# gregspangenberg/shoulder

Measured on AMD Instinct MI355X. Metric: humerus meshes/s end-to-end (all 4 landmarks), higher is better.
Workload: dtype f64 geometry + bf16 UNet

## Files before the change

shoulder_amd/csrc/k_slices.h:

```cpp
#pragma once
#include "sh_demand.h"
#include "sh_scalar.h"
#include "sh_cutmath.h"

namespace sh {

struct __attribute__((aligned(16))) Seg {
  uint32_t s_lo, s_hi, e_lo, e_hi;
};
static_assert(sizeof(Seg) == 16, "Seg must be 16 bytes");
__device__ inline void seg_start_point(const double* __restrict__ vb , uint32_t lo, uint32_t hi, double z, double* x, double* y) {
  const double* pl = vb + 3 * (size_t)lo;
  const double* ph = vb + 3 * (size_t)hi;
  const double dl = pl[2] - z, dh = ph[2] - z;
  const double t = dl / (dl - dh);
  *x = pl[0] + t * (ph[0] - pl[0]);
  *y = pl[1] + t * (ph[1] - pl[1]);
}

__device__ inline unsigned long long enc_f64(double v) {
  unsigned long long b = (unsigned long long)__double_as_longlong(v);
  return (b & 0x8000000000000000ull) ? ~b : (b | 0x8000000000000000ull);
}
__device__ inline double dec_f64(unsigned long long e) {
  unsigned long long b = (e & 0x8000000000000000ull) ? (e & 0x7FFFFFFFFFFFFFFFull) : ~e;
  return __longlong_as_double((long long)b);
}

__global__ void k_transform_verts(const float* __restrict__ verts, const long long* __restrict__ voff,
                                  const double* __restrict__ T, double* __restrict__ vobb,
                                  unsigned long long* __restrict__ zb_enc ) {
  int b = blockIdx.y;
  long long v0 = voff[b], nv = voff[b + 1] - v0;
  const double* Tb = T + 16 * b;
  double zmin = 1e300, zmax = -1e300;
  for (long long i = blockIdx.x * (long long)blockDim.x + threadIdx.x; i < nv; i += (long long)gridDim.x * blockDim.x) {
    const float* p = verts + 3 * (v0 + i);
    double o[3];
    xform_pt(Tb, (double)p[0], (double)p[1], (double)p[2], o);
    double* q = vobb + 3 * (v0 + i);
    q[0] = o[0]; q[1] = o[1]; q[2] = o[2];
    zmin = fmin(zmin, o[2]); zmax = fmax(zmax, o[2]);
  }
  for (int off = 32; off > 0; off >>= 1) {
    zmin = fmin(zmin, __shfl_down(zmin, off));
    zmax = fmax(zmax, __shfl_down(zmax, off));
  }
  if ((threadIdx.x & 63) == 0) {
    atomicMin(&zb_enc[2 * b], enc_f64(zmin));
    atomicMin(&zb_enc[2 * b + 1], ~enc_f64(zmax));
  }
}

__global__ void k_decode_bounds(const unsigned long long* zb_enc, double* zb, int B) {
  int i = blockIdx.x * blockDim.x + threadIdx.x;
  if (i < 2 * B) zb[i] = dec_f64((i & 1) ? ~zb_enc[i] : zb_enc[i]);
}

__device__ inline double np_pairwise_sum(const double* a, int n) {
  if (n < 8) {
    double r = 0.0;
    for (int i = 0; i < n; ++i) r += a[i];
    return r;
  } else if (n <= 128) {
    double r[8];
    for (int k = 0; k < 8; ++k) r[k] = a[k];
    int i;
    for (i = 8; i < n - (n % 8); i += 8)
      for (int k = 0; k < 8; ++k) r[k] += a[i + k];
    double res = ((r[0] + r[1]) + (r[2] + r[3])) + ((r[4] + r[5]) + (r[6] + r[7]));
    for (; i < n; ++i) res += a[i];
    return res;
  } else {
    int n2 = n / 2;
    n2 -= n2 % 8;
    return np_pairwise_sum(a, n2) + np_pairwise_sum(a + n2, n - n2);
  }
}

struct PlaneAux {
  const unsigned long long* zb_enc; double* zb_out;
  int* seg_count; int* nlarge;
  int* ovf_nlist; unsigned long long* ovf_ctr;
};
struct ManyLoops { int* list; int* n; unsigned long long* missed; };
struct SliceSetDev {
  int N, kind, select;
  const double* zb;
  double* zs; double* zeff;
  int* seg_count; Seg* segs;
  double* centroids; double* areas; int* nloops; int* ring_n; double* ring ; double* areas_total ;
  int* nlarge; ManyLoops many; unsigned long long* ovf_missed;
  PlaneAux aux;
};
struct OpenCfg { int mode; double max_gap; int* stats; };

struct SliceSets { SliceSetDev s[2]; int n; const double* vobb; const long long* voff; OpenCfg open; };

__global__ void k_make_planes(SliceSets sets, const double* __restrict__ neck_z, int B) {
  const SliceSetDev& S = sets.s[blockIdx.y];
  const int kind = S.kind, N = S.N;
  const double* zb = S.zb;
  double* zs = S.zs; double* zeff = S.zeff;
  const PlaneAux A = S.aux;
  int b = blockIdx.x;
  if (b >= B) return;
  for (int k = threadIdx.x; k < N; k += blockDim.x) A.seg_count[(size_t)b * N + k] = 0;
  if (b == 0 && threadIdx.x == 0) {
    *A.nlarge = 0;
    if (A.ovf_nlist) { A.ovf_nlist[0] = 0; A.ovf_nlist[1] = 0 ; if (A.ovf_ctr) { A.ovf_ctr[SH_CTR_SEG_USED] = 0ull; A.ovf_ctr[SH_CTR_WORK_USED] = 0ull; } }
  }
  if (kind == 3) {
    if (threadIdx.x == 0) { zs[b] = neck_z[b]; zeff[b] = neck_z[b]; }
    return;
  }
  double zmin, zmax;
  if (A.zb_enc) {
    zmin = dec_f64(A.zb_enc[2 * b]); zmax = dec_f64(~A.zb_enc[2 * b + 1]);
    if (threadIdx.x == 0) { A.zb_out[2 * b] = zmin; A.zb_out[2 * b + 1] = zmax; }
  } else { zmin = zb[2 * b]; zmax = zb[2 * b + 1]; }
  double a, e;
  if (kind == 4) {
    for (int k = threadIdx.x; k < N; k += blockDim.x) { double z = linspace_at(zmin * 0.99, zmax * 0.99, N, k); zs[(size_t)b * N + k] = z; zeff[(size_t)b * N + k] = z; }
    return;
  }
  if (kind == 0) { a = 0.99 * zmax; e = 0.99 * zmin; }
  else if (kind == 1) { a = 0.99 * zmax; e = neck_z[b]; }
  else { a = 0.99 * zmin; e = 0.0; }
  double* z = zs + (size_t)b * N;
  for (int k = threadIdx.x; k < N; k += blockDim.x) z[k] = linspace_at(a, e, N, k);
  __syncthreads();
  __shared__ double z_orig;
  if (threadIdx.x == 0) z_orig = np_pairwise_sum(z, N) / (double)N;
  __syncthreads();
  for (int k = threadIdx.x; k < N; k += blockDim.x) zeff[(size_t)b * N + k] = z_orig + (z[k] - z_orig);
}

#define SH_EMIT_MAXN 640
__global__ void __launch_bounds__(256)
k_slice_emit(const double* __restrict__ vobb, const int* __restrict__ faces,
             const long long* __restrict__ voff, const long long* __restrict__ foff, SliceSets sets) {
  __shared__ int hist[SH_EMIT_MAXN];
  int b = blockIdx.y;
  long long f0 = foff[b], nf = foff[b + 1] - f0;
  const double* vb = vobb + 3 * voff[b];
  const int nsets = sets.n, Ntot = sets.s[0].N + (nsets > 1 ? sets.s[1].N : 0);
  for (long long f_base = blockIdx.x * (long long)blockDim.x; f_base < nf; f_base += (long long)gridDim.x * blockDim.x) {
    for (int k = threadIdx.x; k < Ntot; k += blockDim.x) hist[k] = 0;
    const long long fi = f_base + threadIdx.x;
    const bool live = fi < nf;
    const int* f = faces + 3 * (f0 + (live ? fi : 0));
    int id[3] = {f[0], f[1], f[2]};
    double Z[3];
    for (int k = 0; k < 3; ++k) Z[k] = vb[3 * (size_t)id[k] + 2];
    double fzmin = fmin(Z[0], fmin(Z[1], Z[2])), fzmax = fmax(Z[0], fmax(Z[1], Z[2]));
    int lo_[2] = {1, 1}, hi_[2] = {0, 0};
    for (int si = 0; si < nsets; ++si) {
      const int N = sets.s[si].N;
      const double* zp = sets.s[si].zeff + (size_t)b * N;
      const double z_first = zp[0], z_last = zp[N - 1];
      const double inv_step = (double)(N - 1) / (z_last - z_first);
      double ka = (fzmin - z_first) * inv_step, kb = (fzmax - z_first) * inv_step;
      double klo = fmin(ka, kb), khi = fmax(ka, kb);
      int lo = 1, hi = 0;
      if (live && !(khi < -1.0 || klo > (double)N)) {
        lo = (int)floor(fmax(klo, 0.0)) - 1; hi = (int)ceil(fmin(khi, (double)(N - 1))) + 1;
        lo = lo < 0 ? 0 : lo;
        hi = hi > N - 1 ? N - 1 : hi;
      }
      if (live && N == 1) { lo = 0; hi = 0; }
      lo_[si] = lo; hi_[si] = hi;
    }
    __syncthreads();
    for (int si = 0; si < nsets; ++si) {
      const int N = sets.s[si].N, hoff = si ? sets.s[0].N : 0;
      const double* zp = sets.s[si].zeff + (size_t)b * N;
      for (int k = lo_[si]; k <= hi_[si]; ++k) {
        const double z = zp[k];
        const int s0 = Z[0] - z < -SH_SECTION_TOL ? -1 : 1, s1 = Z[1] - z < -SH_SECTION_TOL ? -1 : 1, s2 = Z[2] - z < -SH_SECTION_TOL ? -1 : 1;
        if (!(s0 == s1 && s1 == s2)) atomicAdd(&hist[hoff + k], 1);
      }
    }
    __syncthreads();
    for (int k = threadIdx.x; k < Ntot; k += blockDim.x) {
      const int n = hist[k];
      if (n > 0) {
        const int si = k >= sets.s[0].N ? 1 : 0, kk = si ? k - sets.s[0].N : k;
        hist[k] = atomicAdd(&sets.s[si].seg_count[(size_t)b * sets.s[si].N + kk], n);
      }
    }
    __syncthreads();
    for (int si = 0; si < nsets; ++si) {
      const int N = sets.s[si].N, hoff = si ? sets.s[0].N : 0;
      const double* zp = sets.s[si].zeff + (size_t)b * N;
      Seg* segs = sets.s[si].segs;
      for (int k = lo_[si]; k <= hi_[si]; ++k) {
        const double z = zp[k];
        double d[3];
        int s[3];
        for (int j = 0; j < 3; ++j) { d[j] = Z[j] - z; s[j] = d[j] < -SH_SECTION_TOL ? -1 : 1; }
        if (s[0] == s[1] && s[1] == s[2]) continue;
        const int slot = atomicAdd(&hist[hoff + k], 1);
        int up = 0, dn = 0;
        for (int j = 0; j < 3; ++j) {
          int jn = (j + 1) % 3;
          if (s[j] == -1 && s[jn] == 1) up = j;
          if (s[j] == 1 && s[jn] == -1) dn = j;
        }
        Seg sg;
        {
          int a = dn, c = (dn + 1) % 3;
          int l = id[a] < id[c] ? a : c, h = id[a] < id[c] ? c : a;
          sg.s_lo = (uint32_t)id[l]; sg.s_hi = (uint32_t)id[h];
        }
        {
          int a = up, c = (up + 1) % 3;
          int l = id[a] < id[c] ? a : c, h = id[a] < id[c] ? c : a;
          sg.e_lo = (uint32_t)id[l]; sg.e_hi = (uint32_t)id[h];
        }
        if (slot < SH_MAXSEG) segs[((size_t)b * N + k) * SH_MAXSEG + slot] = sg;
      }
    }
    __syncthreads();
  }
}

#define SH_LINK_THREADS 256
#define SH_SMALLSEG 384

template <int T>
__device__ inline int bridge_open_chains(const int n, const int cap, const int maxe, unsigned long long* __restrict__ skey,
                                         const unsigned long long* __restrict__ ekey, int* __restrict__ nxt, int* __restrict__ pred,
                                         int* __restrict__ ctl, int* tl, int* hd, int* bt, int* bh, int* mt, int* mh,
                                         double* tx, double* ty, double* hx, double* hy,
                                         const double* __restrict__ vb, const double z, const double max_gap) {
  const int tid = threadIdx.x;
  for (int i = tid; i < n; i += T) pred[i] = 0;
  if (tid < 4) ctl[tid] = 0;
  __syncthreads();
  for (int i = tid; i < n; i += T) if (nxt[i] != i) atomicAdd(&pred[nxt[i]], 1);
  __syncthreads();
  for (int i = tid; i < n; i += T) {
    if (nxt[i] == i) { const int q = atomicAdd(&ctl[0], 1); if (q < maxe) tl[q] = i; }
    if (pred[i] == 0) { const int q = atomicAdd(&ctl[1], 1); if (q < maxe) hd[q] = i; }
  }
  __syncthreads();
  const int nt = ctl[0], nh = ctl[1];
  if (nt > maxe || nh > maxe) return -1;
  for (int q = tid; q < nt; q += T) { const unsigned long long k = ekey[tl[q]]; seg_start_point(vb, (uint32_t)(k >> 32), (uint32_t)k, z, &tx[q], &ty[q]); mt[q] = -1; }
  for (int q = tid; q < nh; q += T) { const unsigned long long k = skey[hd[q]]; seg_start_point(vb, (uint32_t)(k >> 32), (uint32_t)k, z, &hx[q], &hy[q]); mh[q] = -1; }
  for (;;) {
    __syncthreads();
    if (tid == 0) ctl[2] = 0;
    for (int q = tid; q < nt; q += T) {
      int best = -1; double bd = 0.0; unsigned long long bk = 0;
      if (mt[q] < 0)
        for (int h = 0; h < nh; ++h) {
          if (mh[h] >= 0) continue;
          const double dx = tx[q] - hx[h], dy = ty[q] - hy[h];
          const double d = sqrt(dx * dx + dy * dy);
          if (!(d <= max_gap)) continue;
          const unsigned long long k = skey[hd[h]];
          if (best < 0 || d < bd || (d == bd && k < bk)) { best = h; bd = d; bk = k; }
        }
      bt[q] = best;
    }
    for (int q = tid; q < nh; q += T) {
      int best = -1; double bd = 0.0; unsigned long long bk = 0;
      if (mh[q] < 0)
        for (int t = 0; t < nt; ++t) {
          if (mt[t] >= 0) continue;
          const double dx = tx[t] - hx[q], dy = ty[t] - hy[q];
          const double d = sqrt(dx * dx + dy * dy);
          if (!(d <= max_gap)) continue;
          const unsigned long long k = ekey[tl[t]];
          if (best < 0 || d < bd || (d == bd && k < bk)) { best = t; bd = d; bk = k; }
        }
      bh[q] = best;
    }
    __syncthreads();
    for (int q = tid; q < nt; q += T) {
      const int h = bt[q];
      if (h >= 0 && bh[h] == q) { mt[q] = h; mh[h] = q; ctl[2] = 1; }
    }
    __syncthreads();
    if (ctl[2] == 0) break;
  }
  for (int q = tid; q < nt; q += T)
    if (mt[q] >= 0) {
      const int v = n + atomicAdd(&ctl[3], 1);
      if (v < cap) { skey[v] = ekey[tl[q]]; nxt[v] = hd[mt[q]]; nxt[tl[q]] = v; }
    }
  __syncthreads();
  const int nb = ctl[3];
  return n + nb > cap ? -1 : n + nb;
}


template <int CAP, bool OPEN>
__device__ inline void slice_link_plane(const int pl, int N, const int* __restrict__ seg_count, const Seg* __restrict__ segs,
             const double* __restrict__ vobb, const long long* __restrict__ voff, const double* __restrict__ zeff,
             double* __restrict__ centroids, double* __restrict__ areas, int* __restrict__ nloops,
             int* __restrict__ ring_n, double* __restrict__ ring , int select, int* __restrict__ err,
             double* __restrict__ areas_total , ManyLoops many, const OpenCfg oc,
             int* __restrict__ nlarge = nullptr) {
  constexpr int HASH = CAP <= 384 ? 512 : 2048;
  static_assert(HASH * 4 <= CAP * 8 && HASH > CAP, "the hash table lives in bufB");
  __shared__ unsigned long long skey[CAP];
  __shared__ unsigned long long bufA[CAP];
  __shared__ unsigned long long bufB[CAP];
  __shared__ int nxt[CAP], jmpA[CAP], jmpB[CAP], offA[CAP], offB[CAP];
  int* const table = (int*)bufB;
  __shared__ unsigned long long l_key[SH_MAXLOOPS];
  __shared__ int l_start[SH_MAXLOOPS], l_len[SH_MAXLOOPS], l_off[SH_MAXLOOPS];
  __shared__ double l_area[SH_MAXLOOPS], l_sel[SH_MAXLOOPS];
  __shared__ int n_loops, bad;
  __shared__ double bbv[4];

  const int b = pl / N;
  const int tid = threadIdx.x;
  int cnt = seg_count[pl];
  if (CAP == SH_SMALLSEG ? cnt > SH_SMALLSEG : cnt <= SH_SMALLSEG) {
    if (CAP == SH_SMALLSEG && nlarge && tid == 0) atomicAdd(nlarge, 1);
    return;
  }
  if (cnt > SH_MAXSEG) return;
  const int n = cnt;
  if (tid == 0) { n_loops = 0; bad = 0; }
  for (int i = tid; i < HASH; i += SH_LINK_THREADS) table[i] = -1;
  const Seg* sp = segs + (size_t)pl * SH_MAXSEG;
  const double* vb = vobb + 3 * voff[b];
  const double zpl = zeff[pl];
  for (int i = tid; i < n; i += SH_LINK_THREADS) {
    Seg s = sp[i];
    skey[i] = ((unsigned long long)s.s_lo << 32) | s.s_hi;
    bufA[i] = ((unsigned long long)s.e_lo << 32) | s.e_hi;
  }
  __syncthreads();
  if (n < 3 && !(OPEN && n > 0)) {
    if (tid == 0) {
      centroids[2 * (size_t)pl] = 0; centroids[2 * (size_t)pl + 1] = 0; areas[pl] = 0; nloops[pl] = 0; ring_n[pl] = 0;
      if (areas_total) areas_total[pl] = 0;
      else atomicCAS(&err[b], 0, SH_ERR_GEOMETRY_DEV);
    }
    return;
  }
  for (int i = tid; i < n; i += SH_LINK_THREADS) {
    uint32_t h = hash_key64(skey[i]) & (HASH - 1);
    while (atomicCAS(&table[h], -1, i) != -1) h = (h + 1) & (HASH - 1);
  }
  __syncthreads();
  for (int i = tid; i < n; i += SH_LINK_THREADS) {
    unsigned long long k = bufA[i];
    uint32_t h = hash_key64(k) & (HASH - 1);
    int t, found = -1;
    while ((t = table[h]) != -1) {
      if (skey[t] == k) { found = t; break; }
      h = (h + 1) & (HASH - 1);
    }
    if (found < 0) { found = i; bad = 1; }
    nxt[i] = found;
  }
  __syncthreads();
  const bool bridging = OPEN && (bad || n < 3);
  int n2 = n;
  if (bridging) {
    constexpr int E = SH_MAXLOOPS;
    double* pts = (double*)bufB;
    n2 = bridge_open_chains<SH_LINK_THREADS>(n, CAP, E, skey, bufA, nxt, offB, jmpB, jmpA, jmpA + E, jmpA + 2 * E, jmpA + 3 * E, jmpA + 4 * E,
                                             jmpA + 5 * E, pts, pts + E, pts + 2 * E, pts + 3 * E, vb, zpl, oc.max_gap);
    if (n2 < 0) {
      if (tid == 0) {
        if (many.list) many.list[atomicAdd(many.n, 1)] = pl;
        else if (many.missed) atomicExch(many.missed, 1ull);
        else atomicExch(&err[b], SH_ERR_CAPACITY_DEV);
      }
      return;
    }
    if (tid == 0) bad = 0;
  }
  unsigned long long* labA = bufA;
  unsigned long long* labB = bufB;
  int* ja = jmpA; int* jb = jmpB;
  int* ra = offA; int* rb = offB;
  for (int i = tid; i < n2; i += SH_LINK_THREADS) { labA[i] = skey[i]; ja[i] = nxt[i]; ra[i] = 0; }
  __syncthreads();
  for (int span = 1; span < n2; span <<= 1) {
    for (int i = tid; i < n2; i += SH_LINK_THREADS) {
      const int j = ja[i];
      const unsigned long long a = labA[i], c = labA[j];
      const bool own = a <= c;
      labB[i] = own ? a : c;
      rb[i] = own ? ra[i] : span + ra[j];
      jb[i] = ja[j];
    }
    __syncthreads();
    unsigned long long* tl = labA; labA = labB; labB = tl;
    int* tj = ja; ja = jb; jb = tj;
    int* tr = ra; ra = rb; rb = tr;
  }
  for (int i = tid; i < n2; i += SH_LINK_THREADS)
    if (ra[i] == 0 && (!bridging || (nxt[ja[i]] != ja[i] && ra[nxt[i]] >= 2))) {
      int l = atomicAdd(&n_loops, 1);
      if (l < SH_MAXLOOPS) l_start[l] = i;
    }
  __syncthreads();
  if (n_loops > SH_MAXLOOPS) {
    if (tid == 0) {
      if (many.list) many.list[atomicAdd(many.n, 1)] = pl;
      else if (many.missed) atomicExch(many.missed, 1ull);
      else atomicExch(&err[b], SH_ERR_CAPACITY_DEV);
    }
    return;
  }
  const int nl = n_loops;
  if (tid == 0) {
    for (int a = 1; a < nl; ++a) {
      int v = l_start[a]; int c = a - 1;
      while (c >= 0 && skey[l_start[c]] > skey[v]) { l_start[c + 1] = l_start[c]; --c; }
      l_start[c + 1] = v;
    }
    int off = 0;
    for (int l = 0; l < nl; ++l) {
      int s = l_start[l];
      int L = ra[nxt[s]] + 1;
      l_len[l] = L; l_off[l] = off; off += L;
      l_key[l] = skey[s];
    }
    if (off != n && !bridging) bad = 1;
  }
  __syncthreads();
  if (bridging) {
    if (oc.stats)
      for (int i = tid; i < n; i += SH_LINK_THREADS)
        if (nxt[i] == i || nxt[i] >= n) {
          bool kept = false;
          for (int q = 0; q < nl; ++q) kept |= l_key[q] == labA[i];
          atomicAdd(&oc.stats[2 * b + (kept ? 0 : 1)], 1);
        }
    if (nl == 0) {
      if (tid == 0) {
        centroids[2 * (size_t)pl] = 0; centroids[2 * (size_t)pl + 1] = 0; areas[pl] = 0; nloops[pl] = 0; ring_n[pl] = 0;
        if (areas_total) areas_total[pl] = 0;
        else atomicCAS(&err[b], 0, SH_ERR_GEOMETRY_DEV);
      }
      return;
    }
    __syncthreads();
  }
  double* rx = (double*)bufA;
  double* ry = (double*)bufB;
  int my_pos[(CAP + SH_LINK_THREADS - 1) / SH_LINK_THREADS];
  {
    int c = 0;
    for (int i = tid; i < n2; i += SH_LINK_THREADS, ++c) {
      const unsigned long long key = labA[i];
      int l = -1;
      for (int q = 0; q < nl; ++q) if (l_key[q] == key) { l = q; break; }
      const int L = l >= 0 ? l_len[l] : 1;
      const int r = ra[i];
      const int pos = r == 0 ? 0 : L - r;
      my_pos[c] = l < 0 ? -1 : l_off[l] + pos;
    }
  }
  __syncthreads();
  {
    int c = 0;
    for (int i = tid; i < n2; i += SH_LINK_THREADS, ++c)
      if (my_pos[c] >= 0 && my_pos[c] < n2) {
        if (!OPEN || i < n) { const Seg sg = sp[i]; seg_start_point(vb, sg.s_lo, sg.s_hi, zpl, &rx[my_pos[c]], &ry[my_pos[c]]); }
        else { const unsigned long long kv = skey[i]; seg_start_point(vb, (uint32_t)(kv >> 32), (uint32_t)kv, zpl, &rx[my_pos[c]], &ry[my_pos[c]]); }
      }
  }
  __syncthreads();
  const int lane = tid & 63, wave = tid >> 6;
  const int nv = bridging ? l_off[nl - 1] + l_len[nl - 1] : n;
  if (wave == SH_LINK_THREADS / 64 - 1) {
    double x0 = 1e300, x1 = -1e300, y0 = 1e300, y1 = -1e300;
    for (int i = lane; i < nv; i += 64) {
      const double qx = rx[i], qy = ry[i];
      x0 = fmin(x0, qx); x1 = fmax(x1, qx); y0 = fmin(y0, qy); y1 = fmax(y1, qy);
    }
    for (int off = 32; off > 0; off >>= 1) {
      x0 = fmin(x0, __shfl_down(x0, off)); x1 = fmax(x1, __shfl_down(x1, off));
      y0 = fmin(y0, __shfl_down(y0, off)); y1 = fmax(y1, __shfl_down(y1, off));
    }
    if (lane == 0) { bbv[0] = x0; bbv[1] = x1; bbv[2] = y0; bbv[3] = y1; }
  } else {
    for (int l = wave; l < nl; l += SH_LINK_THREADS / 64 - 1) {
      const int o = l_off[l], L = l_len[l];
      double a2 = 0.0, mx = 0.0, my = 0.0;
      for (int q = lane; q < L; q += 64) {
        const int qn = q + 1 == L ? 0 : q + 1;
        a2 += rx[o + q] * ry[o + qn] - rx[o + qn] * ry[o + q];
        mx += rx[o + q]; my += ry[o + q];
      }
      for (int off = 32; off > 0; off >>= 1) { a2 += __shfl_down(a2, off); mx += __shfl_down(mx, off); my += __shfl_down(my, off); }
      if (lane == 0) {
        l_area[l] = 0.5 * a2;
        mx = (mx + rx[o]) / (double)(L + 1); my = (my + ry[o]) / (double)(L + 1);
        l_sel[l] = fabs(mx) + fabs(my);
      }
    }
  }
  __syncthreads();
  int best = 0;
  for (int l = 1; l < nl; ++l) {
    if (select == 0) { if (fabs(l_area[l]) > fabs(l_area[best])) best = l; }
    else { if (l_sel[l] < l_sel[best]) best = l; }
  }
  if (tid == 0) {
    double x0 = bbv[0], x1 = bbv[1], y0 = bbv[2], y1 = bbv[3];
    centroids[2 * (size_t)pl] = 0.5 * (x0 + x1);
    centroids[2 * (size_t)pl + 1] = 0.5 * (y0 + y1);
    int amax = 0;
    for (int l = 1; l < nl; ++l) if (fabs(l_area[l]) > fabs(l_area[amax])) amax = l;
    areas[pl] = fabs(l_area[amax]);
    if (areas_total) {
      double tot = 0.0;
      for (int l = 0; l < nl; ++l) tot += l_area[l];
      areas_total[pl] = fabs(tot);
    }
    nloops[pl] = nl;
    ring_n[pl] = l_len[best];
    if (bad) atomicCAS(&err[b], 0, SH_ERR_GEOMETRY_DEV);
  }
  if (ring) {
    int l = best, o = l_off[l], L = l_len[l];
    bool rev = l_area[l] < 0;
    double* out = ring + (size_t)pl * (SH_MAXSEG + 1) * 2;
    for (int q = tid; q <= L; q += SH_LINK_THREADS) {
      int qq = q == L ? 0 : q;
      int src = rev ? (qq == 0 ? 0 : L - qq) : qq;
      out[2 * q] = rx[o + src];
      out[2 * q + 1] = ry[o + src];
    }
  }
}

template <bool OPEN>
__global__ void __launch_bounds__(SH_LINK_THREADS)
k_slice_link(SliceSets sets, int B, int* __restrict__ err) {
  const int ntot = sets.s[0].N + (sets.n > 1 ? sets.s[1].N : 0);
  int id = (int)blockIdx.x;
  if (B % 8 == 0) { const int x = id & 7, j = id >> 3; id = (x + 8 * (j / ntot)) * ntot + j % ntot; }
  const int b = id / ntot, kk = id - b * ntot;
  const int si = kk >= sets.s[0].N ? 1 : 0;
  const SliceSetDev& S = sets.s[si];
  slice_link_plane<SH_SMALLSEG, OPEN>(b * S.N + (kk - (si ? sets.s[0].N : 0)), S.N, S.seg_count, S.segs, sets.vobb, sets.voff, S.zeff, S.centroids, S.areas, S.nloops, S.ring_n,
                                S.ring, S.select, err, S.areas_total, S.many, sets.open, S.nlarge);
}
template <bool OPEN>
__global__ void __launch_bounds__(SH_LINK_THREADS)
k_slice_link_large(SliceSets sets, int B, int* __restrict__ err) {
  for (int si = 0; si < sets.n; ++si) {
    const SliceSetDev& S = sets.s[si];
    if (*S.nlarge == 0) continue;
    const int nplanes = B * S.N;
    for (int pl = blockIdx.x; pl < nplanes; pl += gridDim.x) {
      const int cnt = S.seg_count[pl];
      if (cnt > SH_MAXSEG && S.ovf_missed && threadIdx.x == 0) atomicExch(S.ovf_missed, 1ull);
      if (cnt <= SH_SMALLSEG || cnt > SH_MAXSEG) continue;
      slice_link_plane<SH_MAXSEG, OPEN>(pl, S.N, S.seg_count, S.segs, sets.vobb, sets.voff, S.zeff, S.centroids, S.areas, S.nloops, S.ring_n, S.ring, S.select, err, S.areas_total, S.many, sets.open);
      __syncthreads();
    }
  }
}

#define SH_RS_THREADS 128
struct RsWant { int keep_all, st_lo, cs_lo, cs_hi; };
template <int CAP>
__device__ inline void resample_polar_plane(const int pl, int N, int M, const int* __restrict__ ring_n, const double* __restrict__ ring,
                 const double* __restrict__ centroids, double* __restrict__ ixy,
                 double* __restrict__ itr_start, double* __restrict__ itr_cs, const long long* __restrict__ ovf_roff, const RsWant W) {
  static_assert(SH_MPROX % SH_RS_THREADS == 0, "whole samples per lane");
  constexpr int NS = SH_MPROX / SH_RS_THREADS;
  __shared__ double rx[CAP + 1], ry[CAP + 1], d[CAP + 1];
  __shared__ int amin_idx;
  __shared__ double wmin[SH_RS_THREADS / 64];
  __shared__ int widx[SH_RS_THREADS / 64];
  const int tid = threadIdx.x;
  const int L = ring_n[pl];
  if (CAP == SH_SMALLSEG ? L > SH_SMALLSEG : L <= SH_SMALLSEG) return;
  if (ovf_roff[pl] >= 0) return;
  const int kpl = pl % N;
  const bool want_st = W.keep_all || kpl >= W.st_lo, want_cs = W.keep_all || (kpl >= W.cs_lo && kpl < W.cs_hi);
  if (!want_st && !want_cs) return;
  const double* rp = ring + (size_t)pl * (SH_MAXSEG + 1) * 2;
  for (int q = tid; q <= L; q += SH_RS_THREADS) { rx[q] = rp[2 * q]; ry[q] = rp[2 * q + 1]; }
  __syncthreads();
  for (int q = 1 + tid; q <= L; q += SH_RS_THREADS) {
    double dx = rx[q] - rx[q - 1], dy = ry[q] - ry[q - 1];
    d[q] = sqrt(dx * dx + dy * dy);
  }
  __syncthreads();
  if (tid == 0) {
    double acc = 0.0;
    d[0] = 0.0;
    int q = 1;
    for (; q + 8 <= L + 1; q += 8) {
      double v[8];
#pragma unroll
      for (int u = 0; u < 8; ++u) v[u] = d[q + u];
#pragma unroll
      for (int u = 0; u < 8; ++u) { acc += v[u]; v[u] = acc; }
#pragma unroll
      for (int u = 0; u < 8; ++u) d[q + u] = v[u];
    }
    for (; q <= L; ++q) { acc += d[q]; d[q] = acc; }
  }
  __syncthreads();
  const double dmax = d[L];
  double sx[NS], sy[NS];
#pragma unroll
  for (int u = 0; u < NS; ++u) {
    const int j = tid + u * SH_RS_THREADS;
    const double t = linspace_at(0.0, dmax, M, j);
    const int n = L + 1;
    if (t < d[0]) { sx[u] = rx[0]; sy[u] = ry[0]; }
    else if (!(t < d[n - 1])) { sx[u] = rx[n - 1]; sy[u] = ry[n - 1]; }
    else {
      int lo = 0, hi = n - 1;
      while (hi - lo > 1) { const int mid = (lo + hi) >> 1; if (t >= d[mid]) lo = mid; else hi = mid; }
      const double x0 = d[lo], fx = rx[lo], fy = ry[lo];
      if (x0 == t) { sx[u] = fx; sy[u] = fy; }
      else {
        const double den = d[lo + 1] - x0;
        sx[u] = (rx[lo + 1] - fx) / den * (t - x0) + fx;
        sy[u] = (ry[lo + 1] - fy) / den * (t - x0) + fy;
      }
    }
  }
  if (W.keep_all) {
    double* oxy = ixy + (size_t)pl * 2 * M;
#pragma unroll
    for (int u = 0; u < NS; ++u) { const int j = tid + u * SH_RS_THREADS; oxy[j] = sx[u]; oxy[M + j] = sy[u]; }
  }
  const double cx = centroids[2 * (size_t)pl], cy = centroids[2 * (size_t)pl + 1];
  for (int pass = 0; pass < 2; ++pass) {
    if (pass == 0 ? !want_st : !want_cs) continue;
    const double ox = pass ? cx : 0.0, oy = pass ? cy : 0.0;
    double best = 1e300;
    int bi = 0x7fffffff;
    double th[NS], rr[NS];
#pragma unroll
    for (int u = 0; u < NS; ++u) {
      const int j = tid + u * SH_RS_THREADS;
      const double x = sx[u] - ox, y = sy[u] - oy;
      th[u] = atan2(y, x);
      rr[u] = sqrt(x * x + y * y);
      if (th[u] < best || (th[u] == best && j < bi)) { best = th[u]; bi = j; }
    }
    for (int off = 32; off > 0; off >>= 1) {
      double ob = __shfl_down(best, off);
      int oi = __shfl_down(bi, off);
      if (ob < best || (ob == best && oi < bi)) { best = ob; bi = oi; }
    }
    if ((tid & 63) == 0) { wmin[tid >> 6] = best; widx[tid >> 6] = bi; }
    __syncthreads();
    if (tid == 0) {
      double bv = wmin[0]; int bx = widx[0];
      for (int w = 1; w < SH_RS_THREADS / 64; ++w)
        if (wmin[w] < bv || (wmin[w] == bv && widx[w] < bx)) { bv = wmin[w]; bx = widx[w]; }
      amin_idx = bx;
    }
    __syncthreads();
    const int k0 = amin_idx;
    double* o = (pass ? itr_cs : itr_start) + (size_t)pl * 2 * M;
#pragma unroll
    for (int u = 0; u < NS; ++u) {
      int dst = tid + u * SH_RS_THREADS - k0; if (dst < 0) dst += M;
      o[dst] = th[u];
      o[M + dst] = rr[u];
    }
    __syncthreads();
  }
}

__global__ void __launch_bounds__(SH_RS_THREADS)
k_resample_polar(int N, int M, const int* __restrict__ ring_n, const double* __restrict__ ring, const double* __restrict__ centroids,
                 double* __restrict__ ixy, double* __restrict__ itr_start, double* __restrict__ itr_cs, const long long* __restrict__ ovf_roff, const RsWant W) {
  resample_polar_plane<SH_SMALLSEG>(blockIdx.x, N, M, ring_n, ring, centroids, ixy, itr_start, itr_cs, ovf_roff, W);
}
__global__ void __launch_bounds__(SH_RS_THREADS)
k_resample_polar_large(int nplanes, int N, int M, const int* __restrict__ ring_n, const double* __restrict__ ring, const double* __restrict__ centroids,
                       double* __restrict__ ixy, double* __restrict__ itr_start, double* __restrict__ itr_cs, const int* __restrict__ nlarge,
                       const long long* __restrict__ ovf_roff, const RsWant W) {
  if (*nlarge == 0) return;
  for (int pl = blockIdx.x; pl < nplanes; pl += gridDim.x) {
    if (ring_n[pl] <= SH_SMALLSEG || ovf_roff[pl] >= 0) continue;
    resample_polar_plane<SH_MAXSEG>(pl, N, M, ring_n, ring, centroids, ixy, itr_start, itr_cs, ovf_roff, W);
    __syncthreads();
  }
}

}
```

Measured before the change: 9158.

## Shrink slice-link shared memory, keep pointer-jumping state in registers, halve block size

The slice-linking kernel now runs 128-thread blocks with occupancy hints. Its shared arrays are consolidated: the double-buffered label, jump and rank arrays become single buffers, with per-thread copies kept in registers and a barrier between read and write in each pointer-jumping step. Segment endpoint vertices are loaded and intersection points computed early, overlapping the hash-table build, instead of re-reading them after ranking. This cuts LDS footprint and raises blocks per CU, at the cost of more registers and an extra barrier per jumping iteration.

```diff
diff --git a/shoulder_amd/csrc/k_slices.h b/shoulder_amd/csrc/k_slices.h
--- a/shoulder_amd/csrc/k_slices.h
+++ b/shoulder_amd/csrc/k_slices.h
@@ -9,13 +9,14 @@
   uint32_t s_lo, s_hi, e_lo, e_hi;
 };
 static_assert(sizeof(Seg) == 16, "Seg must be 16 bytes");
-__device__ inline void seg_start_point(const double* __restrict__ vb , uint32_t lo, uint32_t hi, double z, double* x, double* y) {
-  const double* pl = vb + 3 * (size_t)lo;
-  const double* ph = vb + 3 * (size_t)hi;
+__device__ inline void seg_point_of(const double* pl , const double* ph , double z, double* x, double* y) {
   const double dl = pl[2] - z, dh = ph[2] - z;
   const double t = dl / (dl - dh);
   *x = pl[0] + t * (ph[0] - pl[0]);
   *y = pl[1] + t * (ph[1] - pl[1]);
+}
+__device__ inline void seg_start_point(const double* __restrict__ vb , uint32_t lo, uint32_t hi, double z, double* x, double* y) {
+  seg_point_of(vb + 3 * (size_t)lo, vb + 3 * (size_t)hi, z, x, y);
 }
 
 __device__ inline unsigned long long enc_f64(double v) {
@@ -225,7 +226,7 @@
   }
 }
 
-#define SH_LINK_THREADS 256
+#define SH_LINK_THREADS 128
 #define SH_SMALLSEG 384
 
 template <int T>
@@ -305,12 +306,15 @@
              double* __restrict__ areas_total , ManyLoops many, const OpenCfg oc,
              int* __restrict__ nlarge = nullptr) {
   constexpr int HASH = CAP <= 384 ? 512 : 2048;
-  static_assert(HASH * 4 <= CAP * 8 && HASH > CAP, "the hash table lives in bufB");
+  static_assert(HASH * 4 <= CAP * 8 && HASH > CAP, "the hash table lives in jmp + rk");
+  constexpr int E = SH_MAXLOOPS;
+  static_assert(!OPEN || 6 * E + 4 <= CAP, "bridge mode's chain-end lists live in jmp");
   __shared__ unsigned long long skey[CAP];
-  __shared__ unsigned long long bufA[CAP];
-  __shared__ unsigned long long bufB[CAP];
-  __shared__ int nxt[CAP], jmpA[CAP], jmpB[CAP], offA[CAP], offB[CAP];
-  int* const table = (int*)bufB;
+  __shared__ unsigned long long lab[CAP];
+  __shared__ int nxt[CAP], jr[2 * CAP];
+  __shared__ double open_pts[OPEN ? 4 * E : 1];
+  int* const jmp = jr; int* const rk = jr + CAP;
+  int* const table = jr;
   __shared__ unsigned long long l_key[SH_MAXLOOPS];
   __shared__ int l_start[SH_MAXLOOPS], l_len[SH_MAXLOOPS], l_off[SH_MAXLOOPS];
   __shared__ double l_area[SH_MAXLOOPS], l_sel[SH_MAXLOOPS];
@@ -326,17 +330,13 @@
   }
   if (cnt > SH_MAXSEG) return;
   const int n = cnt;
-  if (tid == 0) { n_loops = 0; bad = 0; }
-  for (int i = tid; i < HASH; i += SH_LINK_THREADS) table[i] = -1;
+  constexpr int PER = (CAP + SH_LINK_THREADS - 1) / SH_LINK_THREADS;
   const Seg* sp = segs + (size_t)pl * SH_MAXSEG;
   const double* vb = vobb + 3 * voff[b];
   const double zpl = zeff[pl];
-  for (int i = tid; i < n; i += SH_LINK_THREADS) {
-    Seg s = sp[i];
-    skey[i] = ((unsigned long long)s.s_lo << 32) | s.s_hi;
-    bufA[i] = ((unsigned long long)s.e_lo << 32) | s.e_hi;
-  }
-  __syncthreads();
+  Seg sg[PER];
+#pragma unroll
+  for (int c = 0; c < PER; ++c) { const int i = tid + c * SH_LINK_THREADS; sg[c] = sp[i < n ? i : (n > 0 ? n - 1 : 0)]; }
   if (n < 3 && !(OPEN && n > 0)) {
     if (tid == 0) {
       centroids[2 * (size_t)pl] = 0; centroids[2 * (size_t)pl + 1] = 0; areas[pl] = 0; nloops[pl] = 0; ring_n[pl] = 0;
@@ -345,13 +345,35 @@
     }
     return;
   }
+  double vl[PER][3], vh[PER][3];
+#pragma unroll
+  for (int c = 0; c < PER; ++c) {
+    const double* pl_ = vb + 3 * (size_t)sg[c].s_lo;
+    const double* ph_ = vb + 3 * (size_t)sg[c].s_hi;
+#pragma unroll
+    for (int k = 0; k < 3; ++k) { vl[c][k] = pl_[k]; vh[c][k] = ph_[k]; }
+  }
+  if (tid == 0) { n_loops = 0; bad = 0; }
+  for (int i = tid; i < HASH; i += SH_LINK_THREADS) table[i] = -1;
+#pragma unroll
+  for (int c = 0; c < PER; ++c) {
+    const int i = tid + c * SH_LINK_THREADS;
+    if (i < n) {
+      skey[i] = ((unsigned long long)sg[c].s_lo << 32) | sg[c].s_hi;
+      lab[i] = ((unsigned long long)sg[c].e_lo << 32) | sg[c].e_hi;
+    }
+  }
+  __syncthreads();
   for (int i = tid; i < n; i += SH_LINK_THREADS) {
     uint32_t h = hash_key64(skey[i]) & (HASH - 1);
     while (atomicCAS(&table[h], -1, i) != -1) h = (h + 1) & (HASH - 1);
   }
+  double px[PER], py[PER];
+#pragma unroll
+  for (int c = 0; c < PER; ++c) seg_point_of(vl[c], vh[c], zpl, &px[c], &py[c]);
   __syncthreads();
   for (int i = tid; i < n; i += SH_LINK_THREADS) {
-    unsigned long long k = bufA[i];
+    unsigned long long k = lab[i];
     uint32_t h = hash_key64(k) & (HASH - 1);
     int t, found = -1;
     while ((t = table[h]) != -1) {
@@ -365,10 +387,9 @@
   const bool bridging = OPEN && (bad || n < 3);
   int n2 = n;
   if (bridging) {
-    constexpr int E = SH_MAXLOOPS;
-    double* pts = (double*)bufB;
-    n2 = bridge_open_chains<SH_LINK_THREADS>(n, CAP, E, skey, bufA, nxt, offB, jmpB, jmpA, jmpA + E, jmpA + 2 * E, jmpA + 3 * E, jmpA + 4 * E,
-                                             jmpA + 5 * E, pts, pts + E, pts + 2 * E, pts + 3 * E, vb, zpl, oc.max_gap);
+    double* pts = open_pts;
+    n2 = bridge_open_chains<SH_LINK_THREADS>(n, CAP, E, skey, lab, nxt, rk, jmp + 6 * E, jmp, jmp + E, jmp + 2 * E, jmp + 3 * E, jmp + 4 * E,
+                                             jmp + 5 * E, pts, pts + E, pts + 2 * E, pts + 3 * E, vb, zpl, oc.max_gap);
     if (n2 < 0) {
       if (tid == 0) {
         if (many.list) many.list[atomicAdd(many.n, 1)] = pl;
@@ -379,28 +400,38 @@
     }
     if (tid == 0) bad = 0;
   }
-  unsigned long long* labA = bufA;
-  unsigned long long* labB = bufB;
-  int* ja = jmpA; int* jb = jmpB;
-  int* ra = offA; int* rb = offB;
-  for (int i = tid; i < n2; i += SH_LINK_THREADS) { labA[i] = skey[i]; ja[i] = nxt[i]; ra[i] = 0; }
-  __syncthreads();
+  unsigned long long la[PER];
+  int jc[PER], rc[PER];
+#pragma unroll
+  for (int c = 0; c < PER; ++c) {
+    const int i = tid + c * SH_LINK_THREADS;
+    la[c] = 0ull; jc[c] = 0; rc[c] = 0;
+    if (i < n2) { la[c] = skey[i]; jc[c] = nxt[i]; lab[i] = la[c]; jmp[i] = jc[c]; rk[i] = 0; }
+  }
+  __syncthreads();
+  const int nper = (n2 + SH_LINK_THREADS - 1) / SH_LINK_THREADS;
   for (int span = 1; span < n2; span <<= 1) {
-    for (int i = tid; i < n2; i += SH_LINK_THREADS) {
-      const int j = ja[i];
-      const unsigned long long a = labA[i], c = labA[j];
-      const bool own = a <= c;
-      labB[i] = own ? a : c;
-      rb[i] = own ? ra[i] : span + ra[j];
-      jb[i] = ja[j];
-    }
-    __syncthreads();
-    unsigned long long* tl = labA; labA = labB; labB = tl;
-    int* tj = ja; ja = jb; jb = tj;
-    int* tr = ra; ra = rb; rb = tr;
+    unsigned long long o[PER] = {};
+    int rj[PER] = {}, jj[PER] = {};
+#pragma unroll
+    for (int c = 0; c < PER; ++c)
+      if (c < nper) { const int j = jc[c]; o[c] = lab[j]; rj[c] = rk[j]; jj[c] = jmp[j]; }
+    __syncthreads();
+#pragma unroll
+    for (int c = 0; c < PER; ++c) {
+      const int i = tid + c * SH_LINK_THREADS;
+      if (i < n2) {
+        const bool own = la[c] <= o[c];
+        la[c] = own ? la[c] : o[c];
+        rc[c] = own ? rc[c] : span + rj[c];
+        jc[c] = jj[c];
+        lab[i] = la[c]; rk[i] = rc[c]; jmp[i] = jc[c];
+      }
+    }
+    __syncthreads();
   }
   for (int i = tid; i < n2; i += SH_LINK_THREADS)
-    if (ra[i] == 0 && (!bridging || (nxt[ja[i]] != ja[i] && ra[nxt[i]] >= 2))) {
+    if (rk[i] == 0 && (!bridging || (nxt[jmp[i]] != jmp[i] && rk[nxt[i]] >= 2))) {
       int l = atomicAdd(&n_loops, 1);
       if (l < SH_MAXLOOPS) l_start[l] = i;
     }
@@ -423,7 +454,7 @@
     int off = 0;
     for (int l = 0; l < nl; ++l) {
       int s = l_start[l];
-      int L = ra[nxt[s]] + 1;
+      int L = rk[nxt[s]] + 1;
       l_len[l] = L; l_off[l] = off; off += L;
       l_key[l] = skey[s];
     }
@@ -435,7 +466,7 @@
       for (int i = tid; i < n; i += SH_LINK_THREADS)
         if (nxt[i] == i || nxt[i] >= n) {
           bool kept = false;
-          for (int q = 0; q < nl; ++q) kept |= l_key[q] == labA[i];
+          for (int q = 0; q < nl; ++q) kept |= l_key[q] == lab[i];
           atomicAdd(&oc.stats[2 * b + (kept ? 0 : 1)], 1);
         }
     if (nl == 0) {
@@ -448,30 +479,31 @@
     }
     __syncthreads();
   }
-  double* rx = (double*)bufA;
-  double* ry = (double*)bufB;
-  int my_pos[(CAP + SH_LINK_THREADS - 1) / SH_LINK_THREADS];
-  {
-    int c = 0;
-    for (int i = tid; i < n2; i += SH_LINK_THREADS, ++c) {
-      const unsigned long long key = labA[i];
+  double* rx = (double*)lab;
+  double* ry = (double*)skey;
+  int my_pos[PER];
+#pragma unroll
+  for (int c = 0; c < PER; ++c) {
+    const int i = tid + c * SH_LINK_THREADS;
+    my_pos[c] = -1;
+    if (i < n2) {
+      const unsigned long long key = lab[i];
       int l = -1;
       for (int q = 0; q < nl; ++q) if (l_key[q] == key) { l = q; break; }
       const int L = l >= 0 ? l_len[l] : 1;
-      const int r = ra[i];
+      const int r = rk[i];
       const int pos = r == 0 ? 0 : L - r;
       my_pos[c] = l < 0 ? -1 : l_off[l] + pos;
-    }
-  }
-  __syncthreads();
-  {
-    int c = 0;
-    for (int i = tid; i < n2; i += SH_LINK_THREADS, ++c)
-      if (my_pos[c] >= 0 && my_pos[c] < n2) {
-        if (!OPEN || i < n) { const Seg sg = sp[i]; seg_start_point(vb, sg.s_lo, sg.s_hi, zpl, &rx[my_pos[c]], &ry[my_pos[c]]); }
-        else { const unsigned long long kv = skey[i]; seg_start_point(vb, (uint32_t)(kv >> 32), (uint32_t)kv, zpl, &rx[my_pos[c]], &ry[my_pos[c]]); }
-      }
-  }
+      if (OPEN && i >= n) {
+        const unsigned long long kv = skey[i];
+        seg_start_point(vb, (uint32_t)(kv >> 32), (uint32_t)kv, zpl, &px[c], &py[c]);
+      }
+    }
+  }
+  __syncthreads();
+#pragma unroll
+  for (int c = 0; c < PER; ++c)
+    if (my_pos[c] >= 0 && my_pos[c] < n2) { rx[my_pos[c]] = px[c]; ry[my_pos[c]] = py[c]; }
   __syncthreads();
   const int lane = tid & 63, wave = tid >> 6;
   const int nv = bridging ? l_off[nl - 1] + l_len[nl - 1] : n;
@@ -539,7 +571,7 @@
 }
 
 template <bool OPEN>
-__global__ void __launch_bounds__(SH_LINK_THREADS)
+__global__ void __launch_bounds__(SH_LINK_THREADS, OPEN ? 6 : 7)
 k_slice_link(SliceSets sets, int B, int* __restrict__ err) {
   const int ntot = sets.s[0].N + (sets.n > 1 ? sets.s[1].N : 0);
   int id = (int)blockIdx.x;
```

Result: faster. 9280 (median of 6 runs) (+1.3%).
